# pingooio/pingoo

Measured on AMD Instinct MI355X. Metric: requests/sec matched (whole node), 1k-rule WAF, higher is better.
Workload: dtype u8

## Files before the change

### pingoo_amd/build.py

```python
from __future__ import annotations

import os
import shutil
import subprocess
import sys

HERE = os.path.dirname(os.path.abspath(__file__))
CSRC = os.path.join(HERE, "csrc")
LIB = os.path.join(HERE, "libpwaf.so")
SOURCES = ["frontend.cpp", "pattern.cpp", "dfa.cpp", "iptrie.cpp", "filter.cpp", "residual.cpp", "residual_jit.cpp", "rtc.cpp", "compile.cpp", "tableplan.cpp", "scanplan.cpp", "loaders.cpp", "batcher.cpp", "async.cpp", "node.cpp", "engine.cpp", "kernels.hip", "records.hip"]
HEADERS = ["frontend.h", "program.h", "kernels.h", "residual.h", "confirm.h", "records.h", "lscan_split.h", "dirtable.h", "georec.h", "tableplan.h", "scanplan.h", "unicode_data.inc", os.path.join("..", "..", "include", "pwaf.h")]


def hipcc() -> str:
    for cand in (os.environ.get("HIPCC"), shutil.which("hipcc"), "/opt/rocm/bin/hipcc"):
        if cand and os.path.exists(cand):
            return cand
    raise RuntimeError("hipcc not found (needed to build pingoo_amd/libpwaf.so)")


EMBED = os.path.join(CSRC, "residual_h.inc")


def embed() -> str:
    text = open(os.path.join(CSRC, "residual.h")).read()
    assert ')RVMH"' not in text
    out = 'R"RVMH(' + text + ')RVMH"\n'
    if not os.path.exists(EMBED) or open(EMBED).read() != out:
        with open(EMBED, "w") as f:
            f.write(out)
    return EMBED


def is_stale(lib: str = LIB) -> bool:
# ... 50 lines not shown
```

### pingoo_amd/csrc/engine.cpp

```cpp
#include <hip/hip_runtime_api.h>

#include <cstdio>
#include <algorithm>
#include <cstring>
#include <map>
#include <memory>
#include <mutex>
#include <string>
#include <type_traits>
#include <unordered_map>
#include <vector>

#include "dirtable.h"
#include "georec.h"
#include "frontend.h"
#include "kernels.h"
#include "lscan_split.h"
#include "program.h"
#include "records.h"
#include "scanplan.h"
#include "tableplan.h"

using namespace pwaf;

// ... 468 lines not shown
    uint32_t n, n_groups, residual_pass, n_passes, bit_words, pair_stride;
    size_t n_slots, ctrl_words;
    uint32_t pool_cap = 0;
    uint32_t *status_word = nullptr;
    bool zero_deferred = false;
    size_t zero_bytes = 0;
    std::vector<pwaf_strcol> cols;
    std::vector<uint32_t> col_bytes;
    std::vector<uint8_t> col_known;
    VerdictArgs v{};
    bool ipres_launched = false, attr_launched = false;
    pwaf_geo *d_geo = nullptr;
    const ListShape *lshapes = nullptr;
    std::vector<uint32_t> filter_index;
    std::vector<FilterArgs> fall;
    std::vector<FilterArgs> by_stride[2];
    std::vector<ConfirmArgs> call;
    std::vector<ListScanArgs> la[2];
    ColPtrChunk ptrs{};
    uint64_t alg_bytes[3] = {0, 0, 0};
    const FilterArgs *d_all = nullptr, *d_s1 = nullptr, *d_s2 = nullptr;
    const ConfirmArgs *d_c = nullptr;
    const ListScanArgs *d_la[2] = {nullptr, nullptr};
    uint32_t *c_plan = nullptr, *l_plan = nullptr;

    BatchRun(pwaf_engine *e_, Scratch &S_, const pwaf_batch &db_, hipStream_t stream_, const std::vector<uint32_t> *col_begin_)
        : e(e_), S(S_), P(*e_->prog.p), db(db_), stream(stream_), col_begin(col_begin_), sw(switches()), prof(e_, stream_), arg_slot{S_, stream_} {
        lshapes = e->list_plan.shapes;
        n = db.n;
        n_groups = (n + 63) / 64;
        residual_pass = (uint32_t)e->groups.size() + (P.fcmp.empty() ? 0u : 1u);
        n_passes = residual_pass + (P.n_residual ? 1u : 0u);
        bit_words = 2 * n_groups;
        pair_stride = std::max(1u, e->n_bit_atoms + e->n_cmp_atoms + e->n_short);
        n_slots = (size_t)std::max(kGapLists, e->n_gated);
        ctrl_words = 2 + n_slots + e->n_filtered;
    }


    int reserve_scratch(bool sync_status) {
        int rc;
        const uint64_t pool_cap64 = std::max<uint64_t>(std::max<uint64_t>(1u << 20, (uint64_t)n * 8), S.pool_entries);
        pool_cap = (uint32_t)std::min<uint64_t>(pool_cap64, 0x7FFFFFF0u);
        S.pool_entries = pool_cap;
        if (!S.status.p) {
            if ((rc = S.status.reserve(8))) return rc;
            HIP_TRY(hipMemsetAsync(S.status.p, 0, 8, stream));
// ... 230 lines not shown
            if (rc) return rc;
        }
        return PWAF_OK;
    }

    int launch_filter_stage() {
        prof.streaming = true;
        const int rc = timed(by_stride[1].empty() ? "filter_s1" : by_stride[0].empty() ? "filter_s2" : "filter_mix", alg_bytes[1] + alg_bytes[2], "filter kernel", [&] {
            return launch_filter(by_stride[0].data(), (uint32_t)by_stride[0].size(), d_s1, by_stride[1].data(), (uint32_t)by_stride[1].size(), d_s2, stream);
        });
        prof.streaming = false;
        return rc;
    }
    int launch_resolve_stage() {
        bool any_list = false;
        for (const DevGroup &d : e->groups) any_list = any_list || (d.filtered && !d.confirm);
        return timed("resolve+compact", 0xFCu, "resolve / compact kernel", [&] {
            const int he = launch_resolve(fall.data(), (uint32_t)fall.size(), d_all, stream);
            return !he && any_list ? launch_compact(fall.data(), (uint32_t)fall.size(), d_all, stream) : he;
        });
    }
    int launch_confirm_stage() {
        if (call.empty()) return PWAF_OK;
        return timed("confirm", 0xF8u, "confirm kernel", [&] { return launch_confirm(call.data(), (uint32_t)call.size(), d_c, c_plan, e->n_cus, stream); });
    }
    int launch_list_scans() {
        uint32_t *plan_at = l_plan;
        for (int phase = 0; phase < 2; phase++) {
            uint32_t first = 0;
            for (const uint32_t cnt : e->lscan_launches[phase]) {
                char nm[48];
                snprintf(nm, sizeof nm, "lscan_x%u", cnt);
                const int rc = timed(nm, 0xFDu, "gated scan kernel", [&] { return launch_scan_gated(la[phase].data() + first, cnt, d_la[phase] + first, plan_at, lshapes[phase], stream); });
                if (rc) return rc;
                plan_at += 2 * cnt + 1;
                first += cnt;
            }
        }
        return PWAF_OK;
    }
    int launch_fcmp_stage() {
        if (P.fcmp.empty()) return PWAF_OK;
        FcmpArgs fa{};
        std::vector<uint32_t> slots;
        for (size_t k = 0; k < P.fcmp.size(); k++) {
            uint32_t sl[2];
            const uint32_t fld[2] = {P.fcmp[k].a, P.fcmp[k].b};
            for (int q = 0; q < 2; q++) {
                size_t at = std::find(slots.begin(), slots.end(), fld[q]) - slots.begin();
                if (at == slots.size()) slots.push_back(fld[q]);
                sl[q] = (uint32_t)at;
            }
            fa.atoms[k] = P.fcmp[k].op | (sl[0] << 8) | (sl[1] << 16);
        }
        for (size_t q = 0; q < slots.size() && q < kMaxFcmpFields; q++) {
            fa.data[q] = cols[slots[q]].data;
            fa.off[q] = cols[slots[q]].offsets;
        }
// ... 315 lines not shown
            size_t planned = 0;
            for (const uint32_t c : e->lscan_launches[phase]) planned += c;
            if (planned != la[phase].size()) return fail(PWAF_E_DEVICE, "list-scan launch plan does not match the batch's descriptors");
        }
        return PWAF_OK;
    }
    void build_column_pointers() {
        if (!P.n_residual) return;
        const size_t nc = e->n_fields;
        ptrs.count = (uint32_t)(2 * nc);
        for (size_t f = 0; f < nc; f++) { ptrs.p[f] = cols[f].data; ptrs.p[nc + f] = cols[f].offsets; }
    }

    int upload_descriptors() {
        int rc;
        struct Part { size_t at; const void *src; size_t bytes; };
        const size_t b_all = fall.size() * sizeof(FilterArgs), b_s1 = by_stride[0].size() * sizeof(FilterArgs), b_s2 = by_stride[1].size() * sizeof(FilterArgs),
                     b_c = call.size() * sizeof(ConfirmArgs), b_l0 = la[0].size() * sizeof(ListScanArgs), b_l1 = la[1].size() * sizeof(ListScanArgs),
                     b_ptrs = (size_t)ptrs.count * sizeof(void *);
        Layout L;
        const Part up[7] = {{L.take(b_all), fall.data(), b_all}, {L.take(b_s1), by_stride[0].data(), b_s1}, {L.take(b_s2), by_stride[1].data(), b_s2}, {L.take(b_c), call.data(), b_c},
                            {L.take(b_l0 + sizeof(ListScanArgs)), la[0].data(), b_l0}, {L.take(b_l1 + sizeof(ListScanArgs)), la[1].data(), b_l1}, {L.take(b_ptrs), ptrs.p, b_ptrs}};
        const size_t up_bytes = L.size();
        const size_t a_cplan = L.take((call.size() + 2) * 4), a_lplan = L.take((lsplit::plan_words(e->lscan_launches[0]) + lsplit::plan_words(e->lscan_launches[1])) * 4);
        if ((rc = S.args.reserve(L.size()))) return rc;
        char *const abase = (char *)S.args.p;
        d_all = (const FilterArgs *)(abase + up[0].at);
        d_s1 = (const FilterArgs *)(abase + up[1].at);
        d_s2 = (const FilterArgs *)(abase + up[2].at);
        d_c = (const ConfirmArgs *)(abase + up[3].at);
        d_la[0] = (const ListScanArgs *)(abase + up[4].at);
        d_la[1] = (const ListScanArgs *)(abase + up[5].at);
        S.res_cols.p = abase + up[6].at;
        c_plan = (uint32_t *)(abase + a_cplan);
        l_plan = (uint32_t *)(abase + a_lplan);
        if (up_bytes) {
            const uint32_t slot = S.arg_next++ % Scratch::kArgSlots;
            if (S.arg_pending[slot]) HIP_TRY(hipEventSynchronize(S.arg_ev[slot]));
            if ((rc = S.arg_slot[slot].reserve(up_bytes))) return rc;
            char *const hb = (char *)S.arg_slot[slot].p;
            for (const Part &p : up)
                if (p.bytes) memcpy(hb + p.at, p.src, p.bytes);
            arg_slot.slot = (int)slot;
            const int he = upload_args_block(hb, S.args.p, up_bytes, zero_deferred ? S.zero_block.p : nullptr, zero_deferred ? zero_bytes : 0, stream);
            if (he) return fail(PWAF_E_DEVICE, std::string("descriptor upload failed: ") + hipGetErrorString((hipError_t)he));
        } else if (zero_deferred) {
            HIP_TRY(hipMemsetAsync(S.zero_block.p, 0, zero_bytes, stream));
        }
        zero_deferred = false;
        return PWAF_OK;
    }
};

int run_pipeline(pwaf_engine *e, Scratch &S, const pwaf_batch &db , pwaf_verdict *d_out, pwaf_counts *d_counts, uint32_t *d_match_idx,
                 uint32_t *d_n_matches, hipStream_t stream, bool totals_known = false, const std::vector<uint32_t> *col_begin = nullptr, bool sync_status = false,
                 pwaf_geo *d_geo = nullptr, const ReportOut *d_rep = nullptr) {
    if (db.n == 0) return PWAF_OK;
    BatchRun b(e, S, db, stream, col_begin);
// ... 1378 lines not shown
```

### pingoo_amd/csrc/kernels.h

```cpp
#pragma once
#include <cstdint>
#include <string>
#include <vector>

#include "program.h"
#include "scanplan.h"

namespace pwaf {

static constexpr int kMaxPasses = 250;
static constexpr int kVerdictPre = 12;
static constexpr uint32_t kDirChunkWords = 32;

static constexpr uint32_t REC_OVERFLOW = 0x80000000u;
struct PoolEntry {
    uint32_t atom;
    uint32_t next;
};

struct ScanArgs {
    const uint8_t *data;
    const uint32_t *off;
    uint32_t n;
    const uint16_t *tab;
    const uint8_t *classmap;
    const uint8_t *umap;
    uint32_t ill_class;
    const SpecialCell *special;
    const uint32_t *list_off;
// ... 85 lines not shown
    uint32_t *pool_count;
    uint32_t pool_cap;
    uint32_t *status;
    const uint32_t *colmask_local;
    uint32_t n_local;
    uint32_t *gate_lists;
    uint32_t *gate_count;
    uint32_t *enq_bits;
    uint32_t enq_words;
    uint32_t shared_bits;
    const uint32_t *dense_flag;
    uint32_t dense_thresh;
};
static constexpr uint32_t kConfirmThreads = 1024;
static constexpr uint32_t kConfirmPoolBytes = 40 * 1024;
constexpr uint32_t confirm_table_bytes(const size_t pool_bytes) { return (uint32_t)pool_bytes & ~3u; }
constexpr bool confirm_tables_fit(const uint32_t n_entries, const uint32_t n_bytes, const uint32_t n_class_words) {
    return (uint64_t)n_entries * 3u + n_bytes / 4u + n_class_words <= kConfirmPoolBytes / 4;
}
struct ConfirmTableDev {
    const ConfirmArgs *c;
    uint32_t count;
};
int launch_confirm(const ConfirmArgs *host, uint32_t count, const ConfirmArgs *dev, uint32_t *plan, uint32_t n_cus, void *stream);

static constexpr uint32_t kStreamSlab = 128 * 1024;
static constexpr uint32_t kStreamIter = 4096;
static constexpr uint32_t kFilterWaves = 4;
static constexpr uint32_t kCompactWords = 2048;
struct FilterArgs {
    const uint8_t *data;
    const uint32_t *off;
    uint32_t n;
    uint32_t total;
    uint32_t slab0;
    uint32_t init;
    uint32_t mul;
    uint32_t stride;
    const uint32_t *table;
    uint32_t n_heads;
    uint32_t head_w[2][4];
    uint32_t head_m[2][4];
    uint32_t head_len[2];
    uint32_t head_code[2];
    uint32_t *rec;
    uint32_t *chunk_bits;
    uint32_t *sub_count;
// ... 156 lines not shown
    uint32_t has_geo;
    uint4 *gpairs;
    uint32_t *ghdr;
    uint32_t pair_stride;
    uint32_t attr_blocks;
    pwaf_verdict *out;
    unsigned long long *counts;
    uint32_t *match_idx;
    uint32_t *n_matches;
    pwaf_rule_hit *hits;
    uint32_t hits_cap;
    uint32_t *n_hits;
    unsigned long long *rule_hits;
    uint32_t *route;
    uint32_t route_base;
};

int launch_scan(const ScanArgs &a, void *stream);
struct GatedTable {
    const ListScanArgs *g;
    uint32_t count;
    uint32_t debug;
};
int launch_scan_gated(const ListScanArgs *host, uint32_t count, const ListScanArgs *dev, uint32_t *plan, const ListShape &shape, void *stream);
int launch_verdict(const VerdictArgs &a, void *stream);
int launch_ipres(const VerdictArgs &a, void *stream);
struct IpresShape {
    uint32_t threads, coarse_bytes, wg_per_cu;
};
IpresShape ipres_shape();
int launch_attr(const VerdictArgs &a, void *stream);
int launch_dir24(const VerdictArgs &a, void *out , void *esc, void *esc_count, void *stream);
struct GeoRecArgs {
    const uint8_t *ip, *ip_is_v6;
    const uint32_t *asn;
    const uint16_t *country;
    uint32_t n, has_geo;
    const uint32_t *root4, *root6, *nodes;
    const GeoRec *recs;
    const uint32_t *chunks, *vals, *summary;
    uint32_t sum_shift, common;
    uint32_t n_cus;
    uint2 *out;
};
int launch_georec(const GeoRecArgs &a, void *stream);
uint32_t scan_lds_bytes(uint32_t n_hot, uint32_t stride, uint32_t n_gate_atoms);
struct VerdictShape {
// ... 8 lines not shown
```

### pingoo_amd/csrc/kernels.hip

```cpp
#include <hip/hip_runtime.h>

#include <cstdlib>
#include <mutex>
#include <set>

#include "confirm.h"
#include "utf8.h"
#include "kernels.h"
#include "residual.h"

namespace pwaf {

static constexpr int kScanThreads = 1024;
static constexpr int kScanWaves = kScanThreads / 64;
static constexpr uint32_t kNone = 0xFFFFFFFFu;

#define PWAF_LDS __attribute__((address_space(3)))
#define PWAF_GLOBAL __attribute__((address_space(1)))
typedef const PWAF_LDS uint16_t *lds_u16_ptr;
typedef const PWAF_GLOBAL uint16_t *glb_u16_ptr;
typedef const PWAF_LDS uint32_t *lds_u32_ptr;
typedef const PWAF_LDS uint8_t *lds_u8_ptr;
typedef unsigned int u32x4 __attribute__((ext_vector_type(4)));
typedef u32x4 u32x4_u __attribute__((aligned(1)));
// ... 141 lines not shown
    return utf8_class(umap, ill_class, b0, next, end - at);
}

__device__ __forceinline__ bool window_has_high(const u32x4 w) { return ((w.x | w.y | w.z | w.w) & 0x80808080u) != 0u; }
__device__ __noinline__ uint32_t cont_class(const uint32_t own_class, const uint32_t ill_class, const PWAF_GLOBAL unsigned char *gdata, const uint32_t at, const uint32_t start, const uint32_t end) {
    const uint32_t back = min(3u, at - start);
    uint32_t prev = 0;
    for (uint32_t d = 1; d <= back; d++) prev |= (uint32_t)gdata[at - d] << (8u * (d - 1u));
    const uint32_t self_next = *reinterpret_cast<const PWAF_GLOBAL uint32_t __attribute__((aligned(1))) *>(gdata + at);
    return utf8_cont_covered(prev, self_next, back, end - at) ? own_class : ill_class;
}

template <class T>
__device__ __forceinline__ T load_descriptor(const T *p) {
    static_assert(sizeof(T) % 4 == 0, "descriptor size");
    typedef uint32_t __attribute__((may_alias)) word_t;
    uint32_t w[sizeof(T) / 4];
    const word_t *s = reinterpret_cast<const word_t *>(p);
#pragma unroll
    for (size_t i = 0; i < sizeof(T) / 4; i++) w[i] = (uint32_t)__builtin_amdgcn_readfirstlane((int)s[i]);
    T out;
    __builtin_memcpy(&out, w, sizeof(T));
    return out;
}

#define PWAF_EMIT(id) h = emit_list(a.list_off, a.list, a.pool, a.pool_count, a.status, a.pool_cap, (id), h)

template <int CH, bool WIDE>
__device__ __forceinline__ void scan_body(const ScanArgs &a) {
    extern __shared__ __align__(16) unsigned char lds[];
    const uint32_t stride2 = a.stride * 2;
    const uint32_t hot_bytes = a.n_hot * stride2;
    const uint32_t hot_elems = hot_bytes >> 1;
    const uint32_t tab_bytes = (hot_bytes + stride2 + 15) & ~15u;
    if ((uint32_t)(uintptr_t)(PWAF_LDS unsigned char *)lds != 0u) __builtin_trap();
    __builtin_amdgcn_s_setprio(3);
    const PWAF_GLOBAL unsigned char *gtab = (const PWAF_GLOBAL unsigned char *)a.tab;
    const PWAF_GLOBAL unsigned char *gdata = (const PWAF_GLOBAL unsigned char *)a.data;
    const PWAF_GLOBAL uint32_t *goff = (const PWAF_GLOBAL uint32_t *)a.off;
    const uint32_t tid = threadIdx.x, wave = wave_index(), lane = tid & 63;

    for (uint32_t i = tid * 16; i < tab_bytes; i += kScanThreads * 16) {
        uint4 v = make_uint4(0xFFFFFFFFu, 0xFFFFFFFFu, 0xFFFFFFFFu, 0xFFFFFFFFu);
        if (i + 16 <= hot_bytes) v = *reinterpret_cast<const uint4 *>(reinterpret_cast<const unsigned char *>(a.tab) + i);
        *reinterpret_cast<uint4 *>(lds + kClsBytes + i) = v;
    }
// ... 195 lines not shown
        }
#pragma unroll
        for (int q = 0; q < CH; q++) w[q] = wn[q];
        n_lo = f_lo;
        n_hi = f_hi;
        n_base = f_base;
    }
}

template <int CH, bool WIDE>
__global__ __launch_bounds__(kScanThreads) void scan_kernel(ScanArgs a) { scan_body<CH, WIDE>(a); }

__device__ __forceinline__ ListOf list_of(const ListScanArgs &a) {
    ListOf l{a.req_list, a.req_list != nullptr ? min(*a.n_list, a.n) : a.n};
    if (a.dense_mode != 0u) {
        const bool dense = *a.dense_flag > a.dense_thresh;
        if (a.dense_mode == 1u && !dense) l.n_l = 0u;
        if (a.dense_mode == 2u && dense) l.n_l = 0u;
        if (a.dense_mode == 3u && dense) l = ListOf{nullptr, a.n};
    }
    return l;
}

__global__ __launch_bounds__(256) void lscan_plan_kernel(GatedTable b, uint32_t *plan , uint32_t n_waves) {
    __shared__ uint32_t part[256];
    __shared__ unsigned long long all_entries;
    const uint32_t t = threadIdx.x;
    uint32_t items = 0;
    const uint32_t n_l = t < b.count ? list_of(b.g[t]).n_l : 0u;
    if (t == 0) all_entries = 0ull;
    __syncthreads();
    if (n_l != 0u) atomicAdd(&all_entries, (unsigned long long)n_l);
    __syncthreads();
    if (t < b.count) {
        const uint32_t room = n_waves > b.count ? n_waves - b.count : 1u;
        const unsigned long long per_wave = (all_entries + room - 1u) / room;
        uint32_t epi = 1;
        while (epi < 16u && epi < per_wave) epi <<= 1;
        while (epi < 64u * kListWalks && (n_l + epi - 1) / epi > n_waves) epi <<= 1;
        items = (n_l + epi - 1) / epi;
        plan[b.count + 1 + t] = epi;
    }
    part[t] = items;
    __syncthreads();
    for (uint32_t d = 1; d < 256; d <<= 1) {
        const uint32_t v = t >= d ? part[t - d] : 0u;
        __syncthreads();
        part[t] += v;
        __syncthreads();
    }
    if (t < b.count) plan[t] = part[t] - items;
    if (t == 0) plan[b.count] = part[255];
}

__device__ __forceinline__ uint32_t list_step_slow(const uint16_t *hot, const PWAF_GLOBAL uint16_t *flat, const uint64_t *delta, const uint32_t state, const uint32_t c,
                                                   const uint32_t stride, const uint32_t n_hot, const uint32_t n_delta) {
    if (state < n_hot) return hot[state * stride + c];
    const uint32_t k = state - n_hot;
    if (k < n_delta) {
        if (c + 2u == stride) return state;
        const uint64_t rec = delta[k];
        const uint32_t lo = (uint32_t)rec, hi = (uint32_t)(rec >> 32);
        if (c == ((lo >> 16) & 0xFFu)) return hi & 0xFFFFu;
        if (c == (lo >> 24)) return hi >> 16;
        return hot[(lo & 0xFFFFu) * stride + c];
    }
    return flat[state * stride + c];
}

template <uint32_t THREADS>
__device__ __forceinline__ void lscan_async(const ListScanArgs &a, const uint16_t *hot, const unsigned char *cls, const uint64_t *delta, uint32_t it, const uint32_t it_end,
                                            const uint32_t first, const uint32_t n_l, const uint32_t hot_elems, const uint32_t epi) {
    const uint32_t ncls = a.n_classes, stride = ncls + 3u;
    const PWAF_GLOBAL unsigned char *gdata = (const PWAF_GLOBAL unsigned char *)a.data;
    const PWAF_GLOBAL uint16_t *flat = (const PWAF_GLOBAL uint16_t *)a.flat;
    auto record_emit = [&](const uint32_t st, Hits &hh) {
// ... 78 lines not shown
                for (uint32_t k = 0; k < 4; k++) {
                    const uint32_t tt = list_step_slow(hot, flat, delta, state, c[k], stride, a.n_hot, a.n_delta);
                    state = tt & 0x7FFFu;
                    if (tt & 0x8000u) record_emit(state, h);
                }
                p += 4u;
            }
        }
        if (live) {
            if (a.end_off[state + 1] != a.end_off[state]) h = emit_list(a.end_off, a.end_list, a.pool, a.pool_count, a.status, a.pool_cap, state, h);
            a.rec[r] = h.ovf != kNone ? (REC_OVERFLOW | h.ovf) : (h.a0 | (h.a1 << 15));
            if (a.colmask_local != nullptr) {
                uint32_t need = 0;
                if ((h.a0 | (h.ovf + 1u)) != 0) need = gate_mask(a.colmask_local, a.pool, h);
                if (a.need_out != nullptr) a.need_out[li] = need;
                need &= ~(a.shared_bits | need_init);
                if (need) enqueue_mask_once(a.gate_lists, a.gate_count, a.n, r, need, a.enq_bits, a.enq_words);
            }
        }
    }
}

template <uint32_t THREADS>
__global__ __launch_bounds__(THREADS, THREADS == 512 ? 6 : 4) void lscan_kernel(GatedTable b, const uint32_t *plan, uint32_t hot_bytes) {
    extern __shared__ uint32_t lscan_lds[];
    __builtin_amdgcn_s_setprio(3);
    if ((uint32_t)(uintptr_t)(PWAF_LDS unsigned char *)lscan_lds != 0u) __builtin_trap();
    const uint32_t total = plan[b.count];
    const uint32_t it0 = (uint32_t)((uint64_t)total * blockIdx.x / gridDim.x), it1 = (uint32_t)((uint64_t)total * (blockIdx.x + 1) / gridDim.x);
    const unsigned char *cls = reinterpret_cast<const unsigned char *>(lscan_lds + (hot_bytes + 16u) / 4);
    const uint16_t *hot = reinterpret_cast<const uint16_t *>(lscan_lds);
    for (uint32_t it = it0; it < it1;) {
        uint32_t ps = 0;
        for (uint32_t lo = 0, hi = b.count; lo + 1 < hi;) {
            const uint32_t mid = (lo + hi) >> 1;
            if (plan[mid] <= it) lo = mid;
            else hi = mid;
            ps = lo;
        }
        const uint32_t first = plan[ps], it_end = min(it1, plan[ps + 1]), epi = plan[b.count + 1 + ps];
        ListScanArgs a = load_descriptor(&b.g[ps]);
        const ListOf lst = list_of(a);
        a.req_list = lst.req_list;
        const uint32_t ncls = a.n_classes, stride = ncls + 3u;
        const uint32_t hot_elems = a.n_hot * stride;
        uint64_t *delta_lds = reinterpret_cast<uint64_t *>(lscan_lds) + (hot_elems * 2u + 2u + 15u) / 16u * 2u;
        __syncthreads();
        {
            const uint4 *src = reinterpret_cast<const uint4 *>(a.flat);
            uint4 *dst = reinterpret_cast<uint4 *>(lscan_lds);
            const uint32_t units = (hot_elems * 2u + 15u) / 16u;
            for (uint32_t k = threadIdx.x; k < units; k += THREADS * 4u) {
                uint4 v[4];
#pragma unroll
                for (uint32_t q = 0; q < 4; q++) v[q] = k + q * THREADS < units ? src[k + q * THREADS] : make_uint4(0u, 0u, 0u, 0u);
#pragma unroll
                for (uint32_t q = 0; q < 4; q++)
                    if (k + q * THREADS < units) dst[k + q * THREADS] = v[q];
            }
            if (threadIdx.x < 64) lscan_lds[(hot_bytes + 16u) / 4 + threadIdx.x] = reinterpret_cast<const uint32_t *>(a.classmap)[threadIdx.x];
            for (uint32_t k = threadIdx.x; k < a.n_delta; k += THREADS) delta_lds[k] = a.delta[k];
        }
        __syncthreads();
// ... 131 lines not shown
                }
#pragma unroll
                for (uint32_t u = 0; u < kListWalks; u++) {
                    if (p[u] < end[u]) p[u] += 16u;
                    w[u] = wn[u];
                }
            }
#pragma unroll
            for (uint32_t u = 0; u < kListWalks; u++) {
                if (!live[u]) continue;
                if (a.end_off[state[u] + 1] != a.end_off[state[u]]) h[u] = emit_list(a.end_off, a.end_list, a.pool, a.pool_count, a.status, a.pool_cap, state[u], h[u]);
                a.rec[r[u]] = h[u].ovf != kNone ? (REC_OVERFLOW | h[u].ovf) : (h[u].a0 | (h[u].a1 << 15));
                if (a.colmask_local != nullptr) {
                    uint32_t need = 0;
                    if ((h[u].a0 | (h[u].ovf + 1u)) != 0) need = gate_mask(a.colmask_local, a.pool, h[u]);
                    if (a.need_out != nullptr) a.need_out[li[u]] = need;
                    need &= ~(a.shared_bits | need_init[u]);
                    if (need) enqueue_mask_once(a.gate_lists, a.gate_count, a.n, r[u], need, a.enq_bits, a.enq_words);
                }
            }
        }
        it = it_end;
    }
}

__global__ __launch_bounds__(256) void confirm_plan_kernel(ConfirmTableDev b, uint32_t *plan ) {
    __shared__ uint32_t part[256];
    const uint32_t t = threadIdx.x;
    uint32_t items = 0;
    if (t < b.count) {
        const ConfirmArgs *pa = &b.c[t];
        const bool dense = pa->dense_flag != nullptr && *pa->dense_flag > pa->dense_thresh;
        items = dense ? 0u : (min(*pa->pair_count, pa->pair_cap) + kConfirmThreads - 1) / kConfirmThreads;
    }
    part[t] = items;
    __syncthreads();
    for (uint32_t d = 1; d < 256; d <<= 1) {
        const uint32_t v = t >= d ? part[t - d] : 0u;
        __syncthreads();
        part[t] += v;
        __syncthreads();
    }
    if (t < b.count) plan[t] = part[t] - items;
    if (t == 0) plan[b.count] = part[255];
}

__device__ __noinline__ void merge_atom(PoolEntry *pool, uint32_t *pool_count, uint32_t *status, uint32_t pool_cap, uint32_t *rec, uint32_t atom) {
    auto rmw_read = [](uint32_t *p) { return atomicOr(p, 0u); };
    auto publish = [&](uint32_t idx, uint32_t at, uint32_t next) {
        const uint32_t t0 = atomicExch(&pool[idx].atom, at), t1 = atomicExch(&pool[idx].next, next);
        asm volatile("" ::"v"(t0), "v"(t1));
    };
    uint32_t old = rmw_read(rec);
    for (;;) {
        uint32_t upd;
        const uint32_t x = atom + 1u;
        if (!(old & REC_OVERFLOW)) {
            const uint32_t a0 = old & 0x7FFFu, a1 = (old >> 15) & 0x7FFFu;
            if (a0 == x || a1 == x) return;
            if (a0 == 0u) upd = old | x;
            else if (a1 == 0u) upd = old | (x << 15);
            else {
                const uint32_t idx = atomicAdd(pool_count, 3u);
                if (idx + 3u > pool_cap) { atomicOr(status, 1u); return; }
                publish(idx, a0 - 1u, kNone);
                publish(idx + 1u, a1 - 1u, idx);
                publish(idx + 2u, atom, idx + 1u);
                upd = REC_OVERFLOW | (idx + 2u);
            }
        } else {
            const uint32_t head = old & ~REC_OVERFLOW;
            for (uint32_t i = head; i != kNone; i = rmw_read(&pool[i].next))
                if (rmw_read(&pool[i].atom) == atom) return;
            const uint32_t idx = atomicAdd(pool_count, 1u);
            if (idx >= pool_cap) { atomicOr(status, 1u); return; }
            publish(idx, atom, head);
            upd = REC_OVERFLOW | idx;
        }
        const uint32_t seen = atomicCAS(rec, old, upd);
        if (seen == old) return;
        old = seen;
    }
}

__global__ __launch_bounds__(kConfirmThreads, 8) void confirm_kernel(ConfirmTableDev b, const uint32_t *plan) {
    __shared__ uint32_t head[kFilterEntries], ftab[kFilterEntries];
    __shared__ uint32_t pool[kConfirmPoolBytes / 4];
    constexpr uint32_t kConfirmQueue = 1024;
    __shared__ uint32_t app_cnt, app_base, app_queue[kConfirmQueue];
    __builtin_amdgcn_s_setprio(3);
    if (threadIdx.x == 0) app_cnt = 0;
    const uint32_t total = plan[b.count];
    const uint32_t it0 = (uint32_t)((uint64_t)total * blockIdx.x / gridDim.x), it1 = (uint32_t)((uint64_t)total * (blockIdx.x + 1) / gridDim.x);
    for (uint32_t it = it0; it < it1;) {
        uint32_t ps = 0;
        for (uint32_t lo = 0, hi = b.count; lo + 1 < hi;) {
            const uint32_t mid = (lo + hi) >> 1;
            if (plan[mid] <= it) lo = mid;
            else hi = mid;
            ps = lo;
        }
        const uint32_t first_item = plan[ps], it_end = min(it1, plan[ps + 1]);
        const ConfirmArgs a = load_descriptor(&b.c[ps]);
        __syncthreads();
        {
            const uint4 *sh = reinterpret_cast<const uint4 *>(a.c_head), *sf = reinterpret_cast<const uint4 *>(a.ftable);
            constexpr uint32_t kPer = kFilterEntries / 4 / kConfirmThreads;
            uint4 vh[kPer], vf[kPer];
#pragma unroll
            for (uint32_t q = 0; q < kPer; q++) { vh[q] = sh[q * kConfirmThreads + threadIdx.x]; vf[q] = sf[q * kConfirmThreads + threadIdx.x]; }
#pragma unroll
            for (uint32_t q = 0; q < kPer; q++) {
                reinterpret_cast<uint4 *>(head)[q * kConfirmThreads + threadIdx.x] = vh[q];
                reinterpret_cast<uint4 *>(ftab)[q * kConfirmThreads + threadIdx.x] = vf[q];
            }
        }
        const uint32_t e_words = a.n_entries * 3u, b_words = a.n_bytes / 4u, c_words = a.n_class_words;
        const bool in_lds = confirm_tables_fit(a.n_entries, a.n_bytes, a.n_class_words);
        const ConfirmEntry *t_entries = a.c_entries;
        const uint8_t *t_bytes = a.c_bytes;
        const uint32_t *t_classes = a.c_classes;
        if (in_lds) {
            const uint32_t *se = reinterpret_cast<const uint32_t *>(a.c_entries), *sb = reinterpret_cast<const uint32_t *>(a.c_bytes);
            for (uint32_t k = threadIdx.x; k < e_words; k += kConfirmThreads) pool[k] = se[k];
            for (uint32_t k = threadIdx.x; k < b_words; k += kConfirmThreads) pool[e_words + k] = sb[k];
// ... 116 lines not shown
#else
    const uint32_t forced_cap = 0;
#endif
    const uint32_t cap = forced_cap ? forced_cap : std::max(1u, a.n_cus);
    if (blocks > cap) blocks = cap;
    if (blocks == 0) blocks = 1;
    void *args[] = {const_cast<ScanArgs *>(&a)};
    hipError_t e = hipLaunchKernel(fn, dim3(blocks), dim3(kScanThreads), args, lds, (hipStream_t)stream);
    return (int)(e != hipSuccess ? e : hipGetLastError());
}

__global__ __launch_bounds__(256) void copy_args_kernel(const uint4 *__restrict__ src, uint4 *__restrict__ dst, uint32_t n16, uint4 *__restrict__ zero, uint32_t z16) {
    for (uint32_t i = blockIdx.x * 256u + threadIdx.x; i < n16; i += gridDim.x * 256u) dst[i] = src[i];
    for (uint32_t i = blockIdx.x * 256u + threadIdx.x; i < z16; i += gridDim.x * 256u) zero[i] = make_uint4(0u, 0u, 0u, 0u);
}
int upload_args_block(const void *host_pinned, void *dev, size_t bytes, void *zero, size_t zero_bytes, void *stream) {
    const uint32_t n16 = (uint32_t)((bytes + 15) / 16), z16 = (uint32_t)(zero_bytes / 16);
    if (n16 == 0 && z16 == 0) return 0;
    const uint32_t blocks = std::max(std::min<uint32_t>((n16 + 255) / 256, 64u), std::min<uint32_t>((z16 + 2047) / 2048, 1024u));
    hipLaunchKernelGGL(copy_args_kernel, dim3(std::max(1u, blocks)), dim3(256), 0, (hipStream_t)stream, (const uint4 *)host_pinned, (uint4 *)dev, n16, (uint4 *)zero, z16);
    return (int)hipGetLastError();
}

int launch_confirm(const ConfirmArgs *host, uint32_t count, const ConfirmArgs *dev, uint32_t *plan, uint32_t n_cus, void *stream) {
    if (count == 0 || host[0].n == 0) return 0;
    if (count > 256) return (int)hipErrorInvalidValue;
    ConfirmTableDev b{dev, count};
    hipLaunchKernelGGL(confirm_plan_kernel, dim3(1), dim3(256), 0, (hipStream_t)stream, b, plan);
    hipError_t e = hipGetLastError();
    if (e != hipSuccess) return (int)e;
    uint64_t max_items = 0;
    for (uint32_t k = 0; k < count; k++) max_items += ((uint64_t)host[k].pair_cap + kConfirmThreads - 1) / kConfirmThreads;
    const uint32_t blocks = (uint32_t)std::min<uint64_t>(max_items, (uint64_t)std::max(1u, n_cus) * 2u);
    const uint32_t *cplan = plan;
    hipLaunchKernelGGL(confirm_kernel, dim3(blocks), dim3(kConfirmThreads), 0, (hipStream_t)stream, b, cplan);
    return (int)hipGetLastError();
}

static const void *lscan_fn(bool wide) { return wide ? reinterpret_cast<const void *>(lscan_kernel<1024>) : reinterpret_cast<const void *>(lscan_kernel<512>); }

int launch_scan_gated(const ListScanArgs *host, uint32_t count, const ListScanArgs *dev, uint32_t *plan, const ListShape &shape, void *stream) {
    if (count == 0 || host[0].n == 0) return 0;
    if (count > 256) return (int)hipErrorInvalidValue;
    GatedTable b{dev, count, 0u};
#ifdef PWAF_PROFILING
    static const uint32_t async_mode = getenv("PWAF_LSCAN_ASYNC") ? (uint32_t)atoi(getenv("PWAF_LSCAN_ASYNC")) : 0u;
    b.debug = async_mode;
#endif
    const uint32_t blocks = std::max(1u, host[0].n_cus) * shape.wg_per_cu;
    hipLaunchKernelGGL(lscan_plan_kernel, dim3(1), dim3(256), 0, (hipStream_t)stream, b, plan, blocks * (shape.threads / 64u));
    hipError_t e = hipGetLastError();
    if (e != hipSuccess) return (int)e;
    const uint32_t *cplan = plan;
    uint32_t hot_bytes = list_hot_bytes(shape);
    void *args[] = {&b, &cplan, &hot_bytes};
    const void *fn = lscan_fn(shape.threads == 1024);
    e = hipLaunchKernel(fn, dim3(blocks), dim3(shape.threads), args, shape.hot_bytes + 16 + 256, (hipStream_t)stream);
    return (int)(e != hipSuccess ? e : hipGetLastError());
}


typedef unsigned short u16x2 __attribute__((ext_vector_type(2)));

template <bool HEADS, int STRIDE>
__device__ __forceinline__ void filter_rows(const FilterArgs &a, const uint32_t blk, const uint32_t wave, const uint32_t lane) {
    const PWAF_GLOBAL unsigned char *gdata = (const PWAF_GLOBAL unsigned char *)a.data;
    const uint32_t rel = blk * kFilterWaves + wave, slab = a.slab0 + rel;
    const uint64_t base64 = (uint64_t)slab * kStreamSlab;
    if (base64 >= a.total) return;
    const uint32_t total = a.total, base0 = (uint32_t)base64, slab_end = (uint32_t)min<uint64_t>(total, base64 + kStreamSlab);
    unsigned long long *my_bits = reinterpret_cast<unsigned long long *>(a.chunk_bits) + (size_t)rel * (kStreamSlab / 1024);
    uint32_t n_hit = 0;
    const uint32_t mul2 = a.mul | (a.mul << 16);
    constexpr uint32_t kRow = 1024;

    auto load_row = [&](const uint32_t b, const uint32_t q) {
        const uint32_t p = b + kRow * q + 16u * lane;
        return *reinterpret_cast<const PWAF_GLOBAL u32x4_u *>(gdata + (p < total ? p : 0u));
    };
    auto dword_at = [&](const uint32_t p) {
// ... 406 lines not shown

__device__ __forceinline__ uint32_t wave_or(uint32_t x) {
#define PWAF_DPP_OR(ctrl, rows) x |= (uint32_t)__builtin_amdgcn_update_dpp(0, (int)x, (ctrl), (rows), 0xF, true)
    PWAF_DPP_OR(0x111, 0xF);
    PWAF_DPP_OR(0x112, 0xF);
    PWAF_DPP_OR(0x114, 0xF);
    PWAF_DPP_OR(0x118, 0xF);
    PWAF_DPP_OR(0x142, 0xA);
    PWAF_DPP_OR(0x143, 0xC);
#undef PWAF_DPP_OR
    return (uint32_t)__builtin_amdgcn_readlane((int)x, 63);
}

#pragma clang diagnostic push
#pragma clang diagnostic ignored "-Winline-asm"
__device__ __forceinline__ void park64(uint32_t &lo, uint32_t &hi, const unsigned long long m, const uint32_t l) {
    asm volatile("s_mov_b32 m0, %3\n\ts_nop 0\n\tv_writelane_b32 %0, %2, m0\n\tv_writelane_b32 %1, %4, m0"
                 : "+v"(lo), "+v"(hi)
                 : "s"((uint32_t)m), "s"(l), "s"((uint32_t)(m >> 32))
                 : "m0");
}
#pragma clang diagnostic pop

__device__ __forceinline__ uint32_t wave_scan_add(uint32_t x) {
#define PWAF_DPP_ADD(ctrl, rows) x += (uint32_t)__builtin_amdgcn_update_dpp(0, (int)x, (ctrl), (rows), 0xF, true)
    PWAF_DPP_ADD(0x111, 0xF);
    PWAF_DPP_ADD(0x112, 0xF);
    PWAF_DPP_ADD(0x114, 0xF);
    PWAF_DPP_ADD(0x118, 0xF);
    PWAF_DPP_ADD(0x142, 0xA);
    PWAF_DPP_ADD(0x143, 0xC);
#undef PWAF_DPP_ADD
    return x;
}

template <uint32_t PARTS>
__global__ __launch_bounds__(256) void resolve_kernel(FilterTable B) {
    __builtin_amdgcn_s_setprio(3);
    constexpr uint32_t kChunks = kStreamSlab / 16, kWords = kChunks / 32;
    constexpr uint32_t kResolveSparse = 128;
    __shared__ uint32_t s_bits[4][kWords], s_rank[4][kWords];
    const FilterArgs *pa = &B.f[blockIdx.y];
    if ((uint64_t)(pa->slab0 + blockIdx.x * 4 / PARTS) * kStreamSlab >= pa->total) return;
    const FilterArgs a = load_descriptor(pa);
    if (a.dense_flag != nullptr && *a.dense_flag > a.dense_thresh) return;
    const uint32_t wave = wave_index(), rel = (blockIdx.x * 4 + wave) / PARTS, part = (blockIdx.x * 4 + wave) % PARTS, slab = a.slab0 + rel, lane = threadIdx.x & 63;
    constexpr uint32_t kPartChunks = kChunks / PARTS;
    if ((uint64_t)slab * kStreamSlab >= a.total) return;
    const uint32_t cnt = a.sub_count[rel];
    if (cnt == 0) return;
    const bool sparse = a.pairs != nullptr && cnt <= kResolveSparse;
    if (sparse && part != 0u) return;
    const uint32_t lo_c = sparse ? 0u : part * kPartChunks, hi_c = sparse ? kChunks : lo_c + kPartChunks;
    const uint32_t *slab_bits = a.chunk_bits + (size_t)rel * kWords;
    uint32_t *bits = s_bits[wave], *rank = s_rank[wave];
#pragma unroll
    for (uint32_t q = 0; q < kWords / 64; q++) bits[q * 64 + lane] = slab_bits[q * 64 + lane];
// ... 1999 lines not shown
```

Measured before the change: 8.127 billion.

## Fold confirm and list-scan planning kernels into the main kernels

After: 8.111 billion. About the same (-0.2%).

```diff
diff --git a/pingoo_amd/build.py b/pingoo_amd/build.py
--- a/pingoo_amd/build.py
+++ b/pingoo_amd/build.py
@@ -9,7 +9,7 @@
 CSRC = os.path.join(HERE, "csrc")
 LIB = os.path.join(HERE, "libpwaf.so")
 SOURCES = ["frontend.cpp", "pattern.cpp", "dfa.cpp", "iptrie.cpp", "filter.cpp", "residual.cpp", "residual_jit.cpp", "rtc.cpp", "compile.cpp", "tableplan.cpp", "scanplan.cpp", "loaders.cpp", "batcher.cpp", "async.cpp", "node.cpp", "engine.cpp", "kernels.hip", "records.hip"]
-HEADERS = ["frontend.h", "program.h", "kernels.h", "residual.h", "confirm.h", "records.h", "lscan_split.h", "dirtable.h", "georec.h", "tableplan.h", "scanplan.h", "unicode_data.inc", os.path.join("..", "..", "include", "pwaf.h")]
+HEADERS = ["frontend.h", "program.h", "kernels.h", "residual.h", "confirm.h", "records.h", "lscan_split.h", "workplan.h", "dirtable.h", "georec.h", "tableplan.h", "scanplan.h", "unicode_data.inc", os.path.join("..", "..", "include", "pwaf.h")]
 
 
 def hipcc() -> str:
diff --git a/pingoo_amd/csrc/engine.cpp b/pingoo_amd/csrc/engine.cpp
--- a/pingoo_amd/csrc/engine.cpp
+++ b/pingoo_amd/csrc/engine.cpp
@@ -514,7 +514,6 @@
     const FilterArgs *d_all = nullptr, *d_s1 = nullptr, *d_s2 = nullptr;
     const ConfirmArgs *d_c = nullptr;
     const ListScanArgs *d_la[2] = {nullptr, nullptr};
-    uint32_t *c_plan = nullptr, *l_plan = nullptr;
 
     BatchRun(pwaf_engine *e_, Scratch &S_, const pwaf_batch &db_, hipStream_t stream_, const std::vector<uint32_t> *col_begin_)
         : e(e_), S(S_), P(*e_->prog.p), db(db_), stream(stream_), col_begin(col_begin_), sw(switches()), prof(e_, stream_), arg_slot{S_, stream_} {
@@ -791,18 +790,17 @@
     }
     int launch_confirm_stage() {
         if (call.empty()) return PWAF_OK;
-        return timed("confirm", 0xF8u, "confirm kernel", [&] { return launch_confirm(call.data(), (uint32_t)call.size(), d_c, c_plan, e->n_cus, stream); });
+        return timed("confirm", 0xF8u, "confirm kernel", [&] { return launch_confirm(call.data(), (uint32_t)call.size(), d_c, e->n_cus, stream); });
     }
     int launch_list_scans() {
-        uint32_t *plan_at = l_plan;
+        static_assert(lsplit::kListLaunchMax == workplan::kMaxDescriptors, "a list-scan launch holds what one thread per descriptor can plan");
         for (int phase = 0; phase < 2; phase++) {
             uint32_t first = 0;
             for (const uint32_t cnt : e->lscan_launches[phase]) {
                 char nm[48];
                 snprintf(nm, sizeof nm, "lscan_x%u", cnt);
-                const int rc = timed(nm, 0xFDu, "gated scan kernel", [&] { return launch_scan_gated(la[phase].data() + first, cnt, d_la[phase] + first, plan_at, lshapes[phase], stream); });
+                const int rc = timed(nm, 0xFDu, "gated scan kernel", [&] { return launch_scan_gated(la[phase].data() + first, cnt, d_la[phase] + first, lshapes[phase], stream); });
                 if (rc) return rc;
-                plan_at += 2 * cnt + 1;
                 first += cnt;
             }
         }
@@ -1164,7 +1162,6 @@
         const Part up[7] = {{L.take(b_all), fall.data(), b_all}, {L.take(b_s1), by_stride[0].data(), b_s1}, {L.take(b_s2), by_stride[1].data(), b_s2}, {L.take(b_c), call.data(), b_c},
                             {L.take(b_l0 + sizeof(ListScanArgs)), la[0].data(), b_l0}, {L.take(b_l1 + sizeof(ListScanArgs)), la[1].data(), b_l1}, {L.take(b_ptrs), ptrs.p, b_ptrs}};
         const size_t up_bytes = L.size();
-        const size_t a_cplan = L.take((call.size() + 2) * 4), a_lplan = L.take((lsplit::plan_words(e->lscan_launches[0]) + lsplit::plan_words(e->lscan_launches[1])) * 4);
         if ((rc = S.args.reserve(L.size()))) return rc;
         char *const abase = (char *)S.args.p;
         d_all = (const FilterArgs *)(abase + up[0].at);
@@ -1174,8 +1171,6 @@
         d_la[0] = (const ListScanArgs *)(abase + up[4].at);
         d_la[1] = (const ListScanArgs *)(abase + up[5].at);
         S.res_cols.p = abase + up[6].at;
-        c_plan = (uint32_t *)(abase + a_cplan);
-        l_plan = (uint32_t *)(abase + a_lplan);
         if (up_bytes) {
             const uint32_t slot = S.arg_next++ % Scratch::kArgSlots;
             if (S.arg_pending[slot]) HIP_TRY(hipEventSynchronize(S.arg_ev[slot]));
diff --git a/pingoo_amd/csrc/kernels.h b/pingoo_amd/csrc/kernels.h
--- a/pingoo_amd/csrc/kernels.h
+++ b/pingoo_amd/csrc/kernels.h
@@ -5,6 +5,7 @@
 
 #include "program.h"
 #include "scanplan.h"
+#include "workplan.h"
 
 namespace pwaf {
 
@@ -136,7 +137,7 @@
     const ConfirmArgs *c;
     uint32_t count;
 };
-int launch_confirm(const ConfirmArgs *host, uint32_t count, const ConfirmArgs *dev, uint32_t *plan, uint32_t n_cus, void *stream);
+int launch_confirm(const ConfirmArgs *host, uint32_t count, const ConfirmArgs *dev, uint32_t n_cus, void *stream);
 
 static constexpr uint32_t kStreamSlab = 128 * 1024;
 static constexpr uint32_t kStreamIter = 4096;
@@ -339,7 +340,8 @@
     uint32_t count;
     uint32_t debug;
 };
-int launch_scan_gated(const ListScanArgs *host, uint32_t count, const ListScanArgs *dev, uint32_t *plan, const ListShape &shape, void *stream);
+static constexpr uint32_t kListPlanWords = (2u * workplan::kMaxDescriptors + 1u + 3u * (workplan::kMaxDescriptors / 64u) + 3u) / 4u * 4u;
+int launch_scan_gated(const ListScanArgs *host, uint32_t count, const ListScanArgs *dev, const ListShape &shape, void *stream);
 int launch_verdict(const VerdictArgs &a, void *stream);
 int launch_ipres(const VerdictArgs &a, void *stream);
 struct IpresShape {
diff --git a/pingoo_amd/csrc/kernels.hip b/pingoo_amd/csrc/kernels.hip
--- a/pingoo_amd/csrc/kernels.hip
+++ b/pingoo_amd/csrc/kernels.hip
@@ -187,6 +187,39 @@
     T out;
     __builtin_memcpy(&out, w, sizeof(T));
     return out;
+}
+
+__device__ __forceinline__ uint32_t wave_scan_add(uint32_t x) {
+#define PWAF_DPP_ADD(ctrl, rows) x += (uint32_t)__builtin_amdgcn_update_dpp(0, (int)x, (ctrl), (rows), 0xF, true)
+    PWAF_DPP_ADD(0x111, 0xF);
+    PWAF_DPP_ADD(0x112, 0xF);
+    PWAF_DPP_ADD(0x114, 0xF);
+    PWAF_DPP_ADD(0x118, 0xF);
+    PWAF_DPP_ADD(0x142, 0xA);
+    PWAF_DPP_ADD(0x143, 0xC);
+#undef PWAF_DPP_ADD
+    return x;
+}
+
+struct PlanWords {
+    const uint32_t *p;
+    __device__ __forceinline__ uint32_t operator[](const uint32_t i) const { return (uint32_t)__builtin_amdgcn_readfirstlane((int)p[i]); }
+};
+__device__ __forceinline__ void plan_prefix(const uint32_t items, const uint32_t count, uint32_t *before, uint32_t *wave_tot) {
+    const uint32_t t = threadIdx.x, wave = t >> 6;
+    uint32_t incl = 0;
+    if (wave <= workplan::kMaxDescriptors / 64u) {
+        incl = wave_scan_add(items);
+        if (wave < workplan::kMaxDescriptors / 64u && (t & 63u) == 63u) wave_tot[wave] = incl;
+    }
+    __syncthreads();
+    if (t <= count) {
+        uint32_t base = 0;
+#pragma unroll
+        for (uint32_t w = 0; w < workplan::kMaxDescriptors / 64u; w++) base += w < wave ? wave_tot[w] : 0u;
+        before[t] = base + incl - items;
+    }
+    __syncthreads();
 }
 
 #define PWAF_EMIT(id) h = emit_list(a.list_off, a.list, a.pool, a.pool_count, a.status, a.pool_cap, (id), h)
@@ -428,36 +461,6 @@
     return l;
 }
 
-__global__ __launch_bounds__(256) void lscan_plan_kernel(GatedTable b, uint32_t *plan , uint32_t n_waves) {
-    __shared__ uint32_t part[256];
-    __shared__ unsigned long long all_entries;
-    const uint32_t t = threadIdx.x;
-    uint32_t items = 0;
-    const uint32_t n_l = t < b.count ? list_of(b.g[t]).n_l : 0u;
-    if (t == 0) all_entries = 0ull;
-    __syncthreads();
-    if (n_l != 0u) atomicAdd(&all_entries, (unsigned long long)n_l);
-    __syncthreads();
-    if (t < b.count) {
-        const uint32_t room = n_waves > b.count ? n_waves - b.count : 1u;
-        const unsigned long long per_wave = (all_entries + room - 1u) / room;
-        uint32_t epi = 1;
-        while (epi < 16u && epi < per_wave) epi <<= 1;
-        while (epi < 64u * kListWalks && (n_l + epi - 1) / epi > n_waves) epi <<= 1;
-        items = (n_l + epi - 1) / epi;
-        plan[b.count + 1 + t] = epi;
-    }
-    part[t] = items;
-    __syncthreads();
-    for (uint32_t d = 1; d < 256; d <<= 1) {
-        const uint32_t v = t >= d ? part[t - d] : 0u;
-        __syncthreads();
-        part[t] += v;
-        __syncthreads();
-    }
-    if (t < b.count) plan[t] = part[t] - items;
-    if (t == 0) plan[b.count] = part[255];
-}
 
 __device__ __forceinline__ uint32_t list_step_slow(const uint16_t *hot, const PWAF_GLOBAL uint16_t *flat, const uint64_t *delta, const uint32_t state, const uint32_t c,
                                                    const uint32_t stride, const uint32_t n_hot, const uint32_t n_delta) {
@@ -582,23 +585,41 @@
 }
 
 template <uint32_t THREADS>
-__global__ __launch_bounds__(THREADS, THREADS == 512 ? 6 : 4) void lscan_kernel(GatedTable b, const uint32_t *plan, uint32_t hot_bytes) {
+__global__ __launch_bounds__(THREADS, THREADS == 512 ? 6 : 4) void lscan_kernel(GatedTable b, uint32_t hot_bytes) {
     extern __shared__ uint32_t lscan_lds[];
     __builtin_amdgcn_s_setprio(3);
     if ((uint32_t)(uintptr_t)(PWAF_LDS unsigned char *)lscan_lds != 0u) __builtin_trap();
-    const uint32_t total = plan[b.count];
-    const uint32_t it0 = (uint32_t)((uint64_t)total * blockIdx.x / gridDim.x), it1 = (uint32_t)((uint64_t)total * (blockIdx.x + 1) / gridDim.x);
+    uint32_t *const plan_before = lscan_lds + (hot_bytes + 16u + 256u) / 4;
+    uint32_t *const plan_epi = plan_before + workplan::kMaxDescriptors + 1u;
+    uint32_t *const plan_entries = plan_epi + workplan::kMaxDescriptors;
+    uint32_t *const plan_tot = plan_entries + 2u * (workplan::kMaxDescriptors / 64u);
+    {
+        const uint32_t t = threadIdx.x, n_waves = gridDim.x * (THREADS / 64u);
+        const uint32_t n_l = t < b.count ? list_of(b.g[t]).n_l : 0u;
+        if (t < workplan::kMaxDescriptors) {
+            const uint32_t lo = wave_scan_add(n_l & 0xFFFFu), hi = wave_scan_add(n_l >> 16);
+            if ((t & 63u) == 63u) { plan_entries[2u * (t >> 6)] = lo; plan_entries[2u * (t >> 6) + 1u] = hi; }
+        }
+        __syncthreads();
+        uint32_t items = 0;
+        if (t < b.count) {
+            unsigned long long all_entries = 0ull;
+#pragma unroll
+            for (uint32_t w = 0; w < workplan::kMaxDescriptors / 64u; w++) all_entries += (unsigned long long)plan_entries[2u * w] + ((unsigned long long)plan_entries[2u * w + 1u] << 16);
+            const uint32_t epi = workplan::list_entries_per_item(all_entries, n_l, n_waves, b.count, 64u * kListWalks);
+            items = workplan::list_items(n_l, epi);
+            plan_epi[t] = epi;
+        }
+        plan_prefix(items, b.count, plan_before, plan_tot);
+    }
+    const PlanWords before{plan_before}, epis{plan_epi};
+    const uint32_t total = before[b.count];
+    const uint32_t it0 = workplan::share_begin(total, blockIdx.x, gridDim.x), it1 = workplan::share_begin(total, blockIdx.x + 1u, gridDim.x);
     const unsigned char *cls = reinterpret_cast<const unsigned char *>(lscan_lds + (hot_bytes + 16u) / 4);
     const uint16_t *hot = reinterpret_cast<const uint16_t *>(lscan_lds);
     for (uint32_t it = it0; it < it1;) {
-        uint32_t ps = 0;
-        for (uint32_t lo = 0, hi = b.count; lo + 1 < hi;) {
-            const uint32_t mid = (lo + hi) >> 1;
-            if (plan[mid] <= it) lo = mid;
-            else hi = mid;
-            ps = lo;
-        }
-        const uint32_t first = plan[ps], it_end = min(it1, plan[ps + 1]), epi = plan[b.count + 1 + ps];
+        const uint32_t ps = workplan::pass_of_item(before, b.count, it);
+        const uint32_t first = before[ps], it_end = min(it1, before[ps + 1u]), epi = epis[ps];
         ListScanArgs a = load_descriptor(&b.g[ps]);
         const ListOf lst = list_of(a);
         a.req_list = lst.req_list;
@@ -776,27 +797,6 @@
         }
         it = it_end;
     }
-}
-
-__global__ __launch_bounds__(256) void confirm_plan_kernel(ConfirmTableDev b, uint32_t *plan ) {
-    __shared__ uint32_t part[256];
-    const uint32_t t = threadIdx.x;
-    uint32_t items = 0;
-    if (t < b.count) {
-        const ConfirmArgs *pa = &b.c[t];
-        const bool dense = pa->dense_flag != nullptr && *pa->dense_flag > pa->dense_thresh;
-        items = dense ? 0u : (min(*pa->pair_count, pa->pair_cap) + kConfirmThreads - 1) / kConfirmThreads;
-    }
-    part[t] = items;
-    __syncthreads();
-    for (uint32_t d = 1; d < 256; d <<= 1) {
-        const uint32_t v = t >= d ? part[t - d] : 0u;
-        __syncthreads();
-        part[t] += v;
-        __syncthreads();
-    }
-    if (t < b.count) plan[t] = part[t] - items;
-    if (t == 0) plan[b.count] = part[255];
 }
 
 __device__ __noinline__ void merge_atom(PoolEntry *pool, uint32_t *pool_count, uint32_t *status, uint32_t pool_cap, uint32_t *rec, uint32_t atom) {
@@ -837,24 +837,29 @@
     }
 }
 
-__global__ __launch_bounds__(kConfirmThreads, 8) void confirm_kernel(ConfirmTableDev b, const uint32_t *plan) {
+__global__ __launch_bounds__(kConfirmThreads, 8) void confirm_kernel(ConfirmTableDev b) {
     __shared__ uint32_t head[kFilterEntries], ftab[kFilterEntries];
     __shared__ uint32_t pool[kConfirmPoolBytes / 4];
     constexpr uint32_t kConfirmQueue = 1024;
     __shared__ uint32_t app_cnt, app_base, app_queue[kConfirmQueue];
     __builtin_amdgcn_s_setprio(3);
     if (threadIdx.x == 0) app_cnt = 0;
-    const uint32_t total = plan[b.count];
-    const uint32_t it0 = (uint32_t)((uint64_t)total * blockIdx.x / gridDim.x), it1 = (uint32_t)((uint64_t)total * (blockIdx.x + 1) / gridDim.x);
+    __shared__ uint32_t plan_before[workplan::kMaxDescriptors + 1], plan_tot[workplan::kMaxDescriptors / 64u];
+    {
+        uint32_t items = 0;
+        if (threadIdx.x < b.count) {
+            const ConfirmArgs *pa = &b.c[threadIdx.x];
+            const bool dense = pa->dense_flag != nullptr && *pa->dense_flag > pa->dense_thresh;
+            items = workplan::confirm_items(dense, *pa->pair_count, pa->pair_cap, kConfirmThreads);
+        }
+        plan_prefix(items, b.count, plan_before, plan_tot);
+    }
+    const PlanWords before{plan_before};
+    const uint32_t total = before[b.count];
+    const uint32_t it0 = workplan::share_begin(total, blockIdx.x, gridDim.x), it1 = workplan::share_begin(total, blockIdx.x + 1u, gridDim.x);
     for (uint32_t it = it0; it < it1;) {
-        uint32_t ps = 0;
-        for (uint32_t lo = 0, hi = b.count; lo + 1 < hi;) {
-            const uint32_t mid = (lo + hi) >> 1;
-            if (plan[mid] <= it) lo = mid;
-            else hi = mid;
-            ps = lo;
-        }
-        const uint32_t first_item = plan[ps], it_end = min(it1, plan[ps + 1]);
+        const uint32_t ps = workplan::pass_of_item(before, b.count, it);
+        const uint32_t first_item = before[ps], it_end = min(it1, before[ps + 1u]);
         const ConfirmArgs a = load_descriptor(&b.c[ps]);
         __syncthreads();
         {
@@ -1017,40 +1022,32 @@
     return (int)hipGetLastError();
 }
 
-int launch_confirm(const ConfirmArgs *host, uint32_t count, const ConfirmArgs *dev, uint32_t *plan, uint32_t n_cus, void *stream) {
+int launch_confirm(const ConfirmArgs *host, uint32_t count, const ConfirmArgs *dev, uint32_t n_cus, void *stream) {
     if (count == 0 || host[0].n == 0) return 0;
-    if (count > 256) return (int)hipErrorInvalidValue;
+    if (count > workplan::kMaxDescriptors) return (int)hipErrorInvalidValue;
     ConfirmTableDev b{dev, count};
-    hipLaunchKernelGGL(confirm_plan_kernel, dim3(1), dim3(256), 0, (hipStream_t)stream, b, plan);
-    hipError_t e = hipGetLastError();
-    if (e != hipSuccess) return (int)e;
     uint64_t max_items = 0;
     for (uint32_t k = 0; k < count; k++) max_items += ((uint64_t)host[k].pair_cap + kConfirmThreads - 1) / kConfirmThreads;
     const uint32_t blocks = (uint32_t)std::min<uint64_t>(max_items, (uint64_t)std::max(1u, n_cus) * 2u);
-    const uint32_t *cplan = plan;
-    hipLaunchKernelGGL(confirm_kernel, dim3(blocks), dim3(kConfirmThreads), 0, (hipStream_t)stream, b, cplan);
+    hipLaunchKernelGGL(confirm_kernel, dim3(blocks), dim3(kConfirmThreads), 0, (hipStream_t)stream, b);
     return (int)hipGetLastError();
 }
 
 static const void *lscan_fn(bool wide) { return wide ? reinterpret_cast<const void *>(lscan_kernel<1024>) : reinterpret_cast<const void *>(lscan_kernel<512>); }
 
-int launch_scan_gated(const ListScanArgs *host, uint32_t count, const ListScanArgs *dev, uint32_t *plan, const ListShape &shape, void *stream) {
+int launch_scan_gated(const ListScanArgs *host, uint32_t count, const ListScanArgs *dev, const ListShape &shape, void *stream) {
     if (count == 0 || host[0].n == 0) return 0;
-    if (count > 256) return (int)hipErrorInvalidValue;
+    if (count > workplan::kMaxDescriptors) return (int)hipErrorInvalidValue;
     GatedTable b{dev, count, 0u};
 #ifdef PWAF_PROFILING
     static const uint32_t async_mode = getenv("PWAF_LSCAN_ASYNC") ? (uint32_t)atoi(getenv("PWAF_LSCAN_ASYNC")) : 0u;
     b.debug = async_mode;
 #endif
     const uint32_t blocks = std::max(1u, host[0].n_cus) * shape.wg_per_cu;
-    hipLaunchKernelGGL(lscan_plan_kernel, dim3(1), dim3(256), 0, (hipStream_t)stream, b, plan, blocks * (shape.threads / 64u));
-    hipError_t e = hipGetLastError();
-    if (e != hipSuccess) return (int)e;
-    const uint32_t *cplan = plan;
     uint32_t hot_bytes = list_hot_bytes(shape);
-    void *args[] = {&b, &cplan, &hot_bytes};
+    void *args[] = {&b, &hot_bytes};
     const void *fn = lscan_fn(shape.threads == 1024);
-    e = hipLaunchKernel(fn, dim3(blocks), dim3(shape.threads), args, shape.hot_bytes + 16 + 256, (hipStream_t)stream);
+    const hipError_t e = hipLaunchKernel(fn, dim3(blocks), dim3(shape.threads), args, hot_bytes + 16 + 256 + kListPlanWords * 4, (hipStream_t)stream);
     return (int)(e != hipSuccess ? e : hipGetLastError());
 }
 
@@ -1503,17 +1500,6 @@
 }
 #pragma clang diagnostic pop
 
-__device__ __forceinline__ uint32_t wave_scan_add(uint32_t x) {
-#define PWAF_DPP_ADD(ctrl, rows) x += (uint32_t)__builtin_amdgcn_update_dpp(0, (int)x, (ctrl), (rows), 0xF, true)
-    PWAF_DPP_ADD(0x111, 0xF);
-    PWAF_DPP_ADD(0x112, 0xF);
-    PWAF_DPP_ADD(0x114, 0xF);
-    PWAF_DPP_ADD(0x118, 0xF);
-    PWAF_DPP_ADD(0x142, 0xA);
-    PWAF_DPP_ADD(0x143, 0xC);
-#undef PWAF_DPP_ADD
-    return x;
-}
 
 template <uint32_t PARTS>
 __global__ __launch_bounds__(256) void resolve_kernel(FilterTable B) {
diff --git a/pingoo_amd/csrc/workplan.h b/pingoo_amd/csrc/workplan.h
--- /dev/null
+++ b/pingoo_amd/csrc/workplan.h
@@ -0,0 +1,45 @@
+#pragma once
+#include <stdint.h>
+
+#if defined(__HIPCC__) || defined(__CUDACC__)
+#define PWAF_WORKPLAN_FN __host__ __device__ inline
+#else
+#define PWAF_WORKPLAN_FN inline
+#endif
+
+namespace pwaf {
+namespace workplan {
+
+static constexpr uint32_t kMaxDescriptors = 256;
+
+PWAF_WORKPLAN_FN uint32_t confirm_items(bool dense, uint32_t pair_count, uint32_t pair_cap, uint32_t threads) {
+    if (dense) return 0u;
+    const uint32_t n_p = pair_count < pair_cap ? pair_count : pair_cap;
+    return (n_p + threads - 1u) / threads;
+}
+
+PWAF_WORKPLAN_FN uint32_t list_room(uint32_t n_waves, uint32_t count) { return n_waves > count ? n_waves - count : 1u; }
+PWAF_WORKPLAN_FN uint32_t list_entries_per_item(uint64_t all_entries, uint32_t n_l, uint32_t n_waves, uint32_t count, uint32_t max_epi) {
+    const uint32_t room = list_room(n_waves, count);
+    const uint64_t per_wave = (all_entries + room - 1u) / room;
+    uint32_t epi = 1;
+    while (epi < 16u && epi < per_wave) epi <<= 1;
+    while (epi < max_epi && (n_l + epi - 1u) / epi > n_waves) epi <<= 1;
+    return epi;
+}
+PWAF_WORKPLAN_FN uint32_t list_items(uint32_t n_l, uint32_t epi) { return (n_l + epi - 1u) / epi; }
+
+PWAF_WORKPLAN_FN uint32_t share_begin(uint32_t total, uint32_t block, uint32_t grid) { return (uint32_t)((uint64_t)total * block / grid); }
+template <class Words>
+PWAF_WORKPLAN_FN uint32_t pass_of_item(const Words &items_before, uint32_t count, uint32_t it) {
+    uint32_t lo = 0;
+    for (uint32_t hi = count; lo + 1u < hi;) {
+        const uint32_t mid = (lo + hi) >> 1;
+        if (items_before[mid] <= it) lo = mid;
+        else hi = mid;
+    }
+    return lo;
+}
+
+}
+}
```
